# probabilists/azula

Hardware: AMD Instinct MI355X
Metric: images/sec (whole node), DDIM-64 256x256 UNet (higher is better)
Workload: dtype f32 (f16x2 split: 2 half pieces per operand, 3 partial products, f32 accumulate)

## Files before the change

azula_amd/_lib.py:

```python

from __future__ import annotations

import ctypes as C
import functools
import os
import threading

import torch

_HERE = os.path.dirname(os.path.abspath(__file__))
LIB_PATH = os.environ.get("AZULA_AMD_LIB") or os.path.join(_HERE, "csrc", "libazula_amd.so")

c_f32p = C.c_void_p
c_stream = C.c_void_p


class AzStepCoef(C.Structure):
    _fields_ = [
        ("c_in", C.c_float),
        ("c_skip", C.c_float),
        ("c_out", C.c_float),
        ("c_time", C.c_float),
        ("alpha_t", C.c_float),
        ("alpha_s", C.c_float),
# ... 412 lines not shown
    "az_rownorm_mod_f32": [vp, vp, vp, vp, vp, i64, i64, i64, i64, i64, i32, f32, c_stream],
    "az_rownorm_mod_h16": [vp, vp, vp, vp, vp, i64, i64, i64, i64, i64, i32, f32, i32, c_stream],
    "az_groupnorm_stats_h16": [vp, vp, vp, i64, i64, i64, i64, i64, i32, i32, i32, c_stream],
    "az_affine_act_h16": [vp, vp, vp, i64, vp, vp, i64, i64, i64, i64, i32, i32, i32, c_stream],
    "az_token_copy_f32": [vp, i64, i64, vp, i64, i64, i64, i64, i64, c_stream],
    "az_token_fill_f32": [vp, i64, i64, i64, vp, i64, vp, i64, i64, c_stream],
    "az_token_fill_h16": [vp, i64, i64, i64, vp, i64, vp, i64, i64, i32, c_stream],
    "az_timestep_embedding_f32": [vp, i64, vp, i64, i64, i32, f32, c_stream],
    "az_linear_small_grouped_f32": [vp, i32, i32, i64, i32, i32, c_stream],
    "az_conv2d_f32": [C.POINTER(AzConvArgs), c_stream],
    "az_conv2d_stem_f32": [C.POINTER(AzConvArgs), c_stream],
    "az_conv2d_bf16_f32": [C.POINTER(AzConvArgs), c_stream],
    "az_conv2d_x3_f32": [C.POINTER(AzConvArgs), c_stream],
    "az_conv2d_f16_f32": [C.POINTER(AzConvArgs), c_stream],
    "az_pack_conv_weight_half_f32": [vp, vp, i32, i32, i32, i32, i32, i32, i32, i32, c_stream],
    "az_pack_conv_weight_x3_f32": [vp, vp, i32, i32, i32, i32, i32, i32, i32, c_stream],
    "az_conv2d_suggest_splitk": [i64, i32, i32, i32],
    "az_conv2d_x3_suggest_splitk": [C.POINTER(AzConvArgs)],
    "az_conv2d_winograd_f32": [C.POINTER(AzConvArgs), c_stream],
    "az_conv2d_winograd_suggest_splitk": [i64, i32, i32, i32, i32],
    "az_winograd_pack_filter_f32": [vp, vp, i32, i32, i32, i32, i32, i32, c_stream],
    "az_conv2d_winograd_x3_f32": [C.POINTER(AzConvArgs), c_stream],
    "az_winograd_pack_filter_x3_f32": [vp, vp, i32, i32, i32, i32, i32, i32, c_stream],
    "az_conv2d_f16x2_f32": [C.POINTER(AzConvArgs), c_stream],
    "az_conv2d_winograd_f16x2_f32": [C.POINTER(AzConvArgs), c_stream],
    "az_pack_conv_weight_f16x2_f32": [vp, vp, i32, i32, i32, i32, i32, i32, i32, f32, c_stream],
    "az_winograd_pack_filter_f16x2_f32": [vp, vp, i32, i32, i32, i32, i32, i32, f32, c_stream],
    "az_f16x2_weight_scale": [f32, i32],
    "az_absmax_f32": [vp, vp, i64, c_stream],
    "az_absmax_from_moments_f32": [vp, vp, i64, c_stream],
    "az_conv2d_winograd4_f32": [C.POINTER(AzConvArgs), c_stream],
    "az_conv2d_winograd4_suggest_splitk": [i64, i32, i32, i32, i32],
    "az_winograd4_pack_filter_f32": [vp, vp, i32, i32, i32, i32, i32, i32, c_stream],
    "az_pack_conv_weight_f32": [vp, vp, i32, i32, i32, i32, i32, i32, i32, c_stream],
    "az_attention_f32": [C.POINTER(AzAttnArgs), c_stream],
    "az_attention_x3_f32": [C.POINTER(AzAttnArgs), c_stream],
    "az_attention_f16x2_f32": [C.POINTER(AzAttnArgs), c_stream],
    "az_attention_bf16_f32": [C.POINTER(AzAttnArgs), c_stream],
    "az_attention_f16_f32": [C.POINTER(AzAttnArgs), c_stream],
    "az_qk_prep_f32": [vp, vp, vp, vp, i64, i64, i32, i32, i64, i64, i64, i64, i64, i64, i32, i32, f32, vp, vp, c_stream],
    "az_qk_prep_bwd_f32": [vp, vp, vp, vp, vp, vp, i64, i64, i32, i32, i64, i64, i64, i64, i64, i64, i64, i64, i64, i32, i32, f32, vp, vp,
                           c_stream],
    "az_attention_bwd_f32": [C.POINTER(AzAttnBwdArgs), c_stream],
    "az_swiglu_f32": [vp, vp, i64, i64, i64, i64, c_stream],
    "az_patchify_f32": [vp, vp, vp, i64, i64, i64, i64, i64, i64, c_stream],
    "az_unpatchify_f32": [vp, vp, i64, i64, i64, i64, i64, i64, c_stream],
# ... 82 lines not shown
```

azula_amd/csrc/conv.hip:

```cpp
#include "conv_shared.h"
#include <cstdio>
#include <cstdlib>
#include <type_traits>

namespace {

constexpr int BM = 128;
constexpr int BN = 128;
constexpr int BK = 32;
constexpr int LDSS = 36;
constexpr int TILE_F = (BM + BN) * LDSS;

#include "igemm_kloop.inc"
struct ConvP {
  AzConvArgs a;
  int npix;
  int cin_s;
  int nkc0;
  int nkc1;
  int nk;
  int kps;
  int tiles_m;
  int tiles_n;
  int asm_loop;
// ... 2524 lines not shown
      else launch_igemm_half(q, half == 2, a->src_dtype != 0, dim3((unsigned)nwg, (unsigned)splitk), st);
    }
  } else
  if (half == 1 || half == 2)
    launch_igemm_half(p, half == 2, a->src_dtype != 0, dim3((unsigned)nwg, (unsigned)splitk), st);
  else if (half == 3)
    hipLaunchKernelGGL(conv_igemm_x3_kernel<false>, dim3((unsigned)nwg, (unsigned)splitk), dim3(256), 0, st, p);
  else if (half == 4)
    hipLaunchKernelGGL(conv_igemm_x3_kernel<true>, dim3((unsigned)nwg, (unsigned)splitk), dim3(256), 0, st, p);
  else if (k16)
    hipLaunchKernelGGL(conv_igemm_kernel<16>, dim3((unsigned)nwg, (unsigned)splitk), dim3(256), 0, st, p);
  else
    hipLaunchKernelGGL(conv_igemm_kernel<32>, dim3((unsigned)nwg, (unsigned)splitk), dim3(256), 0, st, p);
  int rc = az_launch_status();
  if (rc != AZ_OK) return rc;
  if (splitk > 1) {
    p.a.gn_quads = a->gn_quads;
    rc = launch_splitk_reduce(p, st, a->dst_dtype ? half : 0);
  }
  return rc;
}

static int wino_prepare(const AzConvArgs* a, int wk, int64_t ustage_bytes, WinoP& p, int& splitk);

int az_conv2d_winograd_f32(const AzConvArgs* a, az_stream_t stream) {
  WinoP p;
  int splitk = 1;
  const int prc = wino_prepare(a, WK, (int64_t)WU_STAGE * 4, p, splitk);
  if (prc != AZ_OK) return prc;
  hipStream_t st = az_s(stream);
  const int64_t nwg = (int64_t)p.cblocks * p.tblocks;
  {
    static std::atomic<uint64_t> lds_c{0}, lds_s{0};
    hipError_t e = az_max_dynamic_lds((const void*)conv_winograd_kernel<false>, W_LDS_BYTES, lds_c);
    if (e != hipSuccess) return (int)e;
    e = az_max_dynamic_lds((const void*)conv_winograd_kernel<true>, W_LDS_BYTES + W_VOFF_BYTES, lds_s);
    if (e != hipSuccess) return (int)e;
  }
  const char* asm_env = az_ab_env("AZ_WINOGRAD_ASM");
  if ((asm_env && asm_env[0] == '0') || (a->in_affine && a->in_act != 0))
    hipLaunchKernelGGL(conv_winograd_kernel<false>, dim3((unsigned)nwg, (unsigned)splitk), dim3(512), W_LDS_BYTES, st, p);
  else
    hipLaunchKernelGGL(conv_winograd_kernel<true>, dim3((unsigned)nwg, (unsigned)splitk), dim3(512), W_LDS_BYTES + W_VOFF_BYTES, st, p);
  int rc = az_launch_status();
  if (rc != AZ_OK) return rc;
  if (splitk > 1) {
    ConvP cp;
    cp.a = p.a;
    cp.a.gn_quads = a->gn_quads;
    cp.npix = p.npix;
    rc = launch_splitk_reduce(cp, st);
  }
  return rc;
}

static int winograd_x3_entry(const AzConvArgs* a, az_stream_t stream, bool h2);
int az_conv2d_winograd_x3_f32(const AzConvArgs* a, az_stream_t stream) { return winograd_x3_entry(a, stream, false); }
int az_conv2d_winograd_f16x2_f32(const AzConvArgs* a, az_stream_t stream) { return winograd_x3_entry(a, stream, true); }

static int winograd_x3_entry(const AzConvArgs* a, az_stream_t stream, bool h2) {
  WinoP p;
  int splitk = 1;
  const int prc = wino_prepare(a, 16, 16ll * WC * 16 * 3 * 2, p, splitk);
  if (prc != AZ_OK) return prc;
  AZ_REQUIRE(p.tiles_w >= 2, AZ_E_UNSUPPORTED);
  if (h2) AZ_REQUIRE(conv_pow2(a->w_scale), AZ_E_SHAPE);
  p.out_scale = h2 ? 1.f / a->w_scale : 1.f;
  if (h2) AZ_REQUIRE(AZ_ALIGNED16(a->in_absmax0) && AZ_ALIGNED16(a->in_absmax1) && (a->in_absmax0 || !a->in_absmax1), AZ_E_ALIGN);
  hipStream_t st = az_s(stream);
  int rc = azi_winograd_x3_launch(p, (unsigned)splitk, st, h2);
  if (rc != AZ_OK) return rc;
  if (splitk > 1) {
    ConvP cp;
    cp.a = p.a;
    cp.a.gn_quads = a->gn_quads;
    cp.npix = p.npix;
    rc = launch_splitk_reduce(cp, st);
  }
  return rc;
}

static int wino_prepare(const AzConvArgs* a, int wk, int64_t ustage_bytes, WinoP& p, int& splitk) {
  AZ_REQUIRE(a && a->src0 && a->weight && a->dst, AZ_E_NULL);
  AZ_REQUIRE(a->ksize == 3 && a->stride == 1 && a->pad == 1 && !a->aniso && a->src_dtype == 0 && a->dst_dtype == 0, AZ_E_UNSUPPORTED);
  AZ_REQUIRE(a->batch > 0 && a->hin > 0 && a->win > 0 && a->hout == a->hin && a->wout == a->win, AZ_E_SHAPE);
  AZ_REQUIRE(a->c0s > 0 && a->c0s % 4 == 0 && a->c1s % 4 == 0 && a->cout_s > 0 && a->cout_s % 4 == 0, AZ_E_SHAPE);
  AZ_REQUIRE((a->c1s == 0) == (a->src1 == nullptr), AZ_E_SHAPE);
  AZ_REQUIRE((a->act >= 0 && a->act <= 4) || a->act == 6, AZ_E_UNSUPPORTED);
  if (a->act == 6) AZ_REQUIRE(a->res && !a->gate && !a->dst_nchw && !a->gn_quads, AZ_E_UNSUPPORTED);
  if (a->act == 4) AZ_REQUIRE(!a->gate && !a->res && !a->dst_nchw && !a->gn_quads && a->cout_s % 8 == 0, AZ_E_UNSUPPORTED);
  if (a->depth != 0) {
    AZ_REQUIRE(a->depth > 0 && a->batch % a->depth == 0 && a->depth_shift > -a->depth && a->depth_shift < a->depth &&
                   (!a->gate || a->gate_bstride == 0) && (a->depth_wrap == 0 || a->depth_wrap == 1),
               AZ_E_UNSUPPORTED);
    const int64_t tiles_img = (int64_t)((a->hout + 1) / 2) * ((a->wout + 1) / 2);
    const int64_t span = (WT + tiles_img - 1) / tiles_img + 2 + a->depth;
    AZ_REQUIRE(span * a->h0 * a->w0 * a->c0s * 4 < (1ll << 31) && span * a->h1 * a->w1 * a->c1s * 4 < (1ll << 31), AZ_E_SHAPE);
  }
  if (a->in_affine)
    AZ_REQUIRE(!a->src1 && a->c0s % 8 == 0 && (a->up0 == 0 || wk == 16) && (a->in_act == 0 || a->in_act == 1) && AZ_ALIGNED16(a->in_affine) &&
                   (int64_t)a->batch * a->c0s * 8 < (1ll << 31),
               AZ_E_UNSUPPORTED);
// ... 25 lines not shown
  p.a = *a;
  p.npix = (int)npix64;
  p.tiles_h = (a->hout + 1) / 2;
  p.tiles_w = (a->wout + 1) / 2;
  p.ntiles = a->batch * p.tiles_h * p.tiles_w;
  p.nkc0 = (a->c0s + wk - 1) / wk;
  p.nkc1 = (a->c1s + wk - 1) / wk;
  p.nk = p.nkc0 + p.nkc1;
  {
    const int64_t tiles_img = (int64_t)p.tiles_h * p.tiles_w;
    const int64_t span = (WT + tiles_img - 1) / tiles_img + 1;
    AZ_REQUIRE(span * a->h0 * a->w0 * a->c0s * 4 < (1ll << 31), AZ_E_SHAPE);
    AZ_REQUIRE(span * a->h1 * a->w1 * a->c1s * 4 < (1ll << 31), AZ_E_SHAPE);
  }
  splitk = a->splitk;
  if (splitk > p.nk) splitk = p.nk;
  p.kps = (p.nk + splitk - 1) / splitk;
  splitk = (p.nk + p.kps - 1) / p.kps;
  p.a.splitk = splitk;
  AZ_REQUIRE(!a->gn_quads || (a->splitk == 1) == (splitk == 1), AZ_E_UNSUPPORTED);
  if (splitk > 1) p.a.gn_quads = nullptr;
  p.cblocks = (a->cout_s + WC - 1) / WC;
  p.tblocks = (p.ntiles + WT - 1) / WT;
  {
    int env_gt = 0, env_gc = 0;
    if (const char* e = az_ab_env("AZ_WINO_RECT")) sscanf(e, "%d,%d", &env_gt, &env_gc);
    int gt = env_gt > 0 ? env_gt : 8, gc = env_gt > 0 ? (env_gc > 0 ? env_gc : p.cblocks) : (wk == 16 ? 2 : 4);
    while (gc > 1 && p.cblocks % gc) gc >>= 1;
    if (env_gt <= 0) gt = 32 / gc;
    while (gt > 1 && p.tblocks % gt) gt >>= 1;
    if (p.cblocks % gc || p.tblocks % gt) gt = 1, gc = p.cblocks;
    p.gt = gt, p.gc = gc;
  }
  AZ_REQUIRE((int64_t)p.nk * p.cblocks * ustage_bytes <= (1ll << 31), AZ_E_SHAPE);
  return AZ_OK;
}

int az_conv2d_winograd_suggest_splitk(int64_t batch, int32_t hout, int32_t wout, int32_t cout_s, int32_t cin_s) {
  const int64_t tiles = batch * ((hout + 1) / 2) * ((wout + 1) / 2);
  const int64_t blocks = ((tiles + WT - 1) / WT) * ((cout_s + WC - 1) / WC);
  const int64_t nk = (cin_s + WK - 1) / WK;
  int64_t want = (256 + blocks - 1) / blocks;
  int64_t maxs = nk / 8;
  if (maxs < 1) maxs = 1;
  if (want > maxs) want = maxs;
  if (want > 16) want = 16;
  if (blocks >= 192) want = 1;
  return (int)(want < 1 ? 1 : want);
}

int az_conv2d_winograd4_f32(const AzConvArgs* a, az_stream_t stream) {
  AZ_REQUIRE(a && a->src0 && a->weight && a->dst, AZ_E_NULL);
  AZ_REQUIRE(a->ksize == 3 && a->stride == 1 && a->pad == 1 && !a->aniso && a->src_dtype == 0 && a->dst_dtype == 0, AZ_E_UNSUPPORTED);
  AZ_REQUIRE(a->batch > 0 && a->hin > 0 && a->win > 0 && a->hout == a->hin && a->wout == a->win, AZ_E_SHAPE);
  AZ_REQUIRE(a->c0s > 0 && a->c0s % 4 == 0 && a->c1s % 4 == 0 && a->cout_s > 0 && a->cout_s % 4 == 0, AZ_E_SHAPE);
  AZ_REQUIRE((a->c1s == 0) == (a->src1 == nullptr), AZ_E_SHAPE);
// ... 82 lines not shown
```

azula_amd/csrc/conv_shared.h:

```cpp
#pragma once

#include "common.h"

namespace {

typedef float f32x16 __attribute__((ext_vector_type(16)));

__device__ __forceinline__ float4 ld4(const float* p) { return *reinterpret_cast<const float4*>(p); }


typedef unsigned int u32x4 __attribute__((ext_vector_type(4)));

__device__ __forceinline__ float4 buf_ld4(__amdgpu_buffer_rsrc_t rsrc, unsigned voff, unsigned soff) {
  const u32x4 v = __builtin_amdgcn_raw_buffer_load_b128(rsrc, (int)voff, (int)soff, 0);
  return __builtin_bit_cast(float4, v);
}

typedef float f32x2 __attribute__((ext_vector_type(2)));
typedef unsigned int u32x2 __attribute__((ext_vector_type(2)));

__device__ __forceinline__ f32x2 buf_ld2(__amdgpu_buffer_rsrc_t rsrc, unsigned voff, unsigned soff) {
  const u32x2 v = __builtin_amdgcn_raw_buffer_load_b64(rsrc, (int)voff, (int)soff, 0);
  return __builtin_bit_cast(f32x2, v);
}

constexpr unsigned OOB = 0x80000000u;

__device__ __forceinline__ int wrap_coord(int i, int n, int mode) {
  if (mode) {
    i %= n;
    if (i < 0) i += n;
  }
  return i;
}
#define AZ_RSRC_CLAMP 0x80000000ll

__device__ __forceinline__ int az_depth_plane(const AzConvArgs& a, int b, bool& ok) {
  ok = true;
  if (a.depth <= 0) return b;
  const int bd = b % a.depth;
  int sb = bd + a.depth_shift;
  if (a.depth_wrap) sb = sb < 0 ? sb + a.depth : (sb >= a.depth ? sb - a.depth : sb);
  else ok = (unsigned)sb < (unsigned)a.depth;
  return b - bd + sb;
}
__device__ __forceinline__ int az_depth_base(const AzConvArgs& a, int b_first) {
  if (a.depth <= 0) return b_first;
  if (a.depth_wrap) return b_first - b_first % a.depth;
  const int s = b_first + a.depth_shift;
  return s > 0 ? s : 0;
}
// ... 253 lines not shown
    g[i] = z;
    r[i] = z;
    if (n[i] >= 0) epilogue_fetch<IO>(a, n[i], b[i], co, g[i], r[i]);
  }
#pragma unroll
  for (int i = 0; i < NB; ++i)
    if (n[i] >= 0) {
      const float4 f = epilogue_apply_store<IO>(a, n[i], b[i], co, v[i], bv, g[i], r[i]);
      if constexpr (MOM) {
        if (i == 0) mom[0] = f.x;
        const float d0 = f.x - mom[0], d1 = f.y - mom[0], d2 = f.z - mom[0], d3 = f.w - mom[0];
        mom[1] += (d0 + d1) + (d2 + d3);
        mom[2] += (d0 * d0 + d1 * d1) + (d2 * d2 + d3 * d3);
      }
    }
}

template <int IO = 0>
__device__ __forceinline__ void epilogue_store(const AzConvArgs& a, int n, int co, float4 v) {
  epilogue_store_b<IO>(a, n, n / (a.hout * a.wout), co, v);
}


}

struct WinoP {
  AzConvArgs a;
  int npix;
  int tiles_h, tiles_w, ntiles;
  int nkc0, nkc1, nk;
  int kps;
  int cblocks;
  int tblocks;
  int gt, gc;
  float out_scale;
};
```

azula_amd/csrc/wino_x3.hip:

```cpp
#include "conv_shared.h"

#include <cstdlib>
#include <type_traits>

namespace {

typedef __bf16 bf16x8 __attribute__((ext_vector_type(8)));
typedef _Float16 f16x8 __attribute__((ext_vector_type(8)));

constexpr int XT = 64;
constexpr int XC = 64;
constexpr int XK = 16;
constexpr int X_ROW = XK * 4;
constexpr int X_FREQ = XT * X_ROW;
constexpr int X_HALF = 8 * X_FREQ;
constexpr int X_STAGE = 2 * X_HALF;
constexpr int X_SLOTS = 768;
constexpr int X_SLOT = 64;
constexpr int X_DOFF1 = X_STAGE + X_SLOTS * X_SLOT;
constexpr int X_OT = 2 * XC + 4;
constexpr int X_EPI_BYTES = (4 * XT * X_OT + 3 * XT + 384) * 4;
constexpr int X_LDS_BYTES = X_DOFF1 + 512 * 32 > X_EPI_BYTES ? X_DOFF1 + 512 * 32 : X_EPI_BYTES;
static_assert(X_LDS_BYTES >= X_DOFF1 + 512 * 32 && X_LDS_BYTES >= 4 * 128 * 64 * 4, "the epilogue reuses the K loop's LDS");
constexpr int XU_STEP_BYTES = 16 * XC * XK * 3 * 2;
static_assert(4 * X_SLOTS <= 6 * 512, "six staging pieces per thread");
static_assert(X_LDS_BYTES <= 160 * 1024, "one workgroup per CU");

template <int AFF, bool TAIL, bool H2 = false>
__global__ __launch_bounds__(512, 2) void conv_winograd_x3_kernel(WinoP p) {
  extern __shared__ __attribute__((aligned(16))) float wsm[];
  char* const smem = reinterpret_cast<char*>(wsm);
  const AzConvArgs& a = p.a;
  const int tid = threadIdx.x;
  const int lane = tid & 63;
  const int wave = tid >> 6;
  const int wxi = wave & 3;
  const int wk = wave >> 2;
  const int l31 = lane & 31;
  const int h = lane >> 5;

  const int nwg = gridDim.x;
  const int bid = blockIdx.x;
  const int xq = nwg >> 3, xr = nwg & 7, xcd = bid & 7;
  const int wg = (xcd < xr ? xcd * (xq + 1) : xr * (xq + 1) + (xcd - xr) * xq) + (bid >> 3);
  const int rsz = p.gt * p.gc;
  const int rect = wg / rsz, rin = wg - rect * rsz;
  const int rcols = p.cblocks / p.gc;
  const int rrow = rect / rcols;
  const int rin_c = rin / p.gt;
  const int tb = rrow * p.gt + (rin - rin_c * p.gt);
  const int cb = (rect - rrow * rcols) * p.gc + rin_c;
  const int t0 = tb * XT;
  const int tiles_img = p.tiles_h * p.tiles_w;
  const int b_first = t0 / tiles_img;

  const int kt_begin = blockIdx.y * p.kps;
  const int kt_end = min(p.nk, kt_begin + p.kps);
  const float pin = H2 ? az_f16x2_in_scale(a.in_absmax0, a.in_absmax1, 4.f, lane) : 1.f;
  const float pin2k = pin * 2048.f;

  const int64_t s0_elems = (int64_t)a.h0 * a.w0 * a.c0s;
  const int64_t s1_elems = (int64_t)a.h1 * a.w1 * a.c1s;
  const int b_base = az_depth_base(a, b_first);
  auto clamp_bytes = [](int64_t e) { return (unsigned)(e <= 0 ? 0 : (e * 4 > AZ_RSRC_CLAMP ? AZ_RSRC_CLAMP : e * 4)); };
  const __amdgpu_buffer_rsrc_t rw = __builtin_amdgcn_make_buffer_rsrc(
      (void*)a.weight, 0, (unsigned)((int64_t)p.nk * p.cblocks * XU_STEP_BYTES), 0x00020000);
  const __amdgpu_buffer_rsrc_t rs0 = __builtin_amdgcn_make_buffer_rsrc(
      (void*)(a.src0 + b_base * s0_elems), 0, clamp_bytes((a.batch - b_base) * s0_elems), 0x00020000);
  const __amdgpu_buffer_rsrc_t rs1 = __builtin_amdgcn_make_buffer_rsrc(
      (void*)(a.src1 ? a.src1 + b_base * s1_elems : a.src0), 0, a.src1 ? clamp_bytes((a.batch - b_base) * s1_elems) : 0u, 0x00020000);

  const int vj = tid >> 3;
  const int vq = tid & 7;
  int v_b = -1, v_ih0 = 0, v_iw0 = 0;
  bool v_dok = true;
  {
    const int t = t0 + vj;
    if (t < p.ntiles) {
      const int b = t / tiles_img;
      const int r = t - b * tiles_img;
      const int th = r / p.tiles_w;
      v_b = b - b_first;
      v_ih0 = 2 * th - 1;
      v_iw0 = 2 * (r - th * p.tiles_w) - 1;
      (void)az_depth_plane(a, b, v_dok);
    }
  }
  const int tw0 = (t0 % tiles_img) % p.tiles_w;
  const int nseg = (XT - 1 + tw0) / p.tiles_w + 1;
  const int nslots = 8 * (XT + nseg);
  const int ndma = (4 * nslots + 511) >> 9;
  auto seg_of = [&](int g, int& js, int& len) {
    js = max(0, g * p.tiles_w - tw0);
    len = min(XT, (g + 1) * p.tiles_w - tw0) - js;
  };
  auto fdiv = [](int x, int d) {
    int q = (int)((float)x * __builtin_amdgcn_rcpf((float)d));
    int r = x - q * d;
    q += r >= d ? 1 : (r < 0 ? -1 : 0);
    return q;
  };
  unsigned doff[6];
  auto dma_offsets = [&](int src) {
    const int cs = src ? a.c1s : a.c0s;
    const int up = src ? a.up1 : a.up0;
    const int hs = src ? a.h1 : a.h0;
    const int ws = src ? a.w1 : a.w0;
    const int row0 = t0 / p.tiles_w;
#pragma unroll
    for (int m = 0; m < 6; ++m) {
      const int L = m * 512 + tid;
      const int s = L >> 2;
      const int g = fdiv((s >> 3) + tw0, p.tiles_w + 1);
      int js, len;
      seg_of(g, js, len);
      const int RS = 2 * len + 2;
      const int o = s - 8 * (js + g);
      const int r = fdiv(o, RS);
      const int x = o - r * RS;
      const int grow = row0 + g;
      const int b = fdiv(grow, p.tiles_h);
      const int th = grow - b * p.tiles_h;
      const int tws = g == 0 ? tw0 : 0;
      bool dok = true;
      const int bs = az_depth_plane(a, b, dok) - b_base;
      const int ih = wrap_coord(2 * th - 1 + r, a.hin, a.pad_mode);
      const int iw = wrap_coord(2 * tws - 1 + x, a.win, a.pad_mode);
      const bool ok = s < nslots && b < a.batch && dok && (unsigned)ih < (unsigned)a.hin && (unsigned)iw < (unsigned)a.win;
      doff[m] = ok ? (unsigned)((((bs * hs + (ih >> up)) * ws + (iw >> up)) * cs + (L & 3) * 4) * 4) : OOB;
    }
  };
  uint4* const park1 = reinterpret_cast<uint4*>(smem + X_DOFF1 + tid * 32);
  int cur_src = 0;
  auto switch_source = [&]() __attribute__((always_inline)) {
    cur_src = 1;
    const uint4 lo = park1[0], hi = park1[1];
    doff[0] = lo.x, doff[1] = lo.y, doff[2] = lo.z, doff[3] = lo.w, doff[4] = hi.x, doff[5] = hi.y;
  };
  if (a.src1) {
    dma_offsets(1);
    park1[0] = make_uint4(doff[0], doff[1], doff[2], doff[3]);
    park1[1] = make_uint4(doff[4], doff[5], 0u, 0u);
  }
  dma_offsets(0);
  if (kt_begin >= p.nkc0) switch_source();
  int pj_s, pj_len;
  seg_of(fdiv(vj + tw0, p.tiles_w), pj_s, pj_len);
  const int prow = (2 * pj_len + 2) * X_SLOT;
  const char* const patch = smem + X_STAGE + (8 * (pj_s + fdiv(vj + tw0, p.tiles_w)) + 2 * (vj - pj_s)) * X_SLOT + vq * 8;
  unsigned vmask = 0;
  if constexpr (AFF != 0) {
#pragma unroll
    for (int r = 0; r < 4; ++r)
#pragma unroll
      for (int c = 0; c < 4; ++c) {
        const int ih = wrap_coord(v_ih0 + r, a.hin, a.pad_mode), iw = wrap_coord(v_iw0 + c, a.win, a.pad_mode);
        if (v_b >= 0 && v_dok && (unsigned)ih < (unsigned)a.hin && (unsigned)iw < (unsigned)a.win) vmask |= 1u << (r * 4 + c);
      }
  }

  f32x2 rv[16];
  float4 gq[6];
  auto gl = [&](int kt, int m) __attribute__((always_inline)) {
    if (m < 5 || m < ndma) {
      const bool src1 = kt >= p.nkc0;
      const int kc = src1 ? kt - p.nkc0 : kt;
      const __amdgpu_buffer_rsrc_t r = src1 ? rs1 : rs0;
      unsigned off = doff[m];
      if constexpr (TAIL) off = kc * XK + (tid & 3) * 4 < (src1 ? a.c1s : a.c0s) ? off : OOB;
      gq[m] = buf_ld4(r, off, (unsigned)(kc * XK * 4));
    }
  };
  auto gs = [&](int m) __attribute__((always_inline)) {
    if (m < 5 || m < ndma) *reinterpret_cast<float4*>(smem + X_STAGE + ((m * 512 + tid) >> 2) * X_SLOT + (tid & 3) * 16) = gq[m];
  };
  auto patch_rows = [&](int kt, int r0, int r1) __attribute__((always_inline)) {
#pragma unroll
    for (int r = r0; r < r1; ++r)
#pragma unroll
      for (int c = 0; c < 4; ++c) rv[4 * r + c] = *reinterpret_cast<const f32x2*>(patch + r * prow + c * X_SLOT);
  };
  const __amdgpu_buffer_rsrc_t raf = __builtin_amdgcn_make_buffer_rsrc(
      (void*)(AFF != 0 ? a.in_affine : nullptr), 0, AFF != 0 ? (unsigned)(2 * a.batch * a.c0s * 4) : 0u, 0x00020000);
  const unsigned af_voff = (unsigned)(((b_first + (v_b < 0 ? 0 : v_b)) * a.c0s + vq * 2) * 4);
  const unsigned af_shift = (unsigned)(a.batch * a.c0s * 4);
  f32x2 af_sc = {0.f, 0.f}, af_sh = {0.f, 0.f};
  auto affine_load = [&](int kt) __attribute__((always_inline)) {
    if constexpr (AFF != 0) {
      const bool kv = !TAIL || kt * XK + vq * 2 < a.c0s;
      af_sc = buf_ld2(raf, kv ? af_voff : OOB, (unsigned)(kt * XK * 4));
      af_sh = buf_ld2(raf, kv ? af_voff : OOB, (unsigned)(kt * XK * 4) + af_shift);
    }
  };
  auto affine = [&]() __attribute__((always_inline)) {
    if constexpr (AFF != 0) {
#pragma unroll
      for (int i = 0; i < 16; ++i) {
// ... 259 lines not shown
    __syncthreads();
    if (wk == 0) {
      float* zbuf = wsm + wxi * (XT * X_OT);
#pragma unroll
      for (int th = 0; th < 2; ++th)
#pragma unroll
        for (int ch = 0; ch < 2; ++ch) {
          float* zrow = zbuf + (th * 32 + l31) * X_OT + ch * 32 + 4 * h;
          const f32x16& z0 = acc[2 * ch + th];
          const f32x16& z1 = acc[4 + 2 * ch + th];
#pragma unroll
          for (int g = 0; g < 4; ++g) {
            *reinterpret_cast<float4*>(zrow + 8 * g) = make_float4(z0[4 * g], z0[4 * g + 1], z0[4 * g + 2], z0[4 * g + 3]);
            *reinterpret_cast<float4*>(zrow + XC + 8 * g) = make_float4(z1[4 * g], z1[4 * g + 1], z1[4 * g + 2], z1[4 * g + 3]);
          }
        }
    }
  }
  int* tinfo = reinterpret_cast<int*>(wsm + 4 * XT * X_OT);
  if (wave < 2 && h == 0) {
    const int tl = wave * 32 + l31;
    const int t = t0 + tl;
    int n00 = -1, fl = 0, b = 0;
    if (t < p.ntiles) {
      b = t / tiles_img;
      const int rr = t - b * tiles_img;
      const int th = rr / p.tiles_w;
      const int tw = rr - th * p.tiles_w;
      n00 = (b * a.hout + 2 * th) * a.wout + 2 * tw;
      fl = (2 * th + 1 < a.hout ? 1 : 0) | (2 * tw + 1 < a.wout ? 2 : 0);
    }
    tinfo[tl] = n00;
    tinfo[XT + tl] = fl;
    tinfo[2 * XT + tl] = b;
  }
  __syncthreads();
  const int cq = tid & 15;
  const int co = cb * XC + cq * 4;
  if (co >= a.cout_s) return;
  int on[8], ob[8];
  float4 ov[8];
#pragma unroll
  for (int it = 0; it < 8; ++it) {
    const int row = (it * 512 + tid) >> 4;
    const int tile = row >> 2, px = row & 3;
    const int n00 = tinfo[tile], fl = tinfo[XT + tile];
    ob[it] = tinfo[2 * XT + tile];
// ... 21 lines not shown
    am = am + 0.5f * d;
    a2 = (a2 + b2) + d * d * half_n;
  };
  chan(am, a2, __shfl_xor(am, 16), __shfl_xor(a2, 16), 16.f);
  chan(am, a2, __shfl_xor(am, 32), __shfl_xor(a2, 32), 32.f);
  float* sh = reinterpret_cast<float*>(tinfo + 3 * XT);
  if (lane < 16) {
    sh[wave * 16 + lane] = am;
    sh[128 + wave * 16 + lane] = a2;
  }
  __syncthreads();
  if (tid < 16) {
    float wm[8], w2[8];
#pragma unroll
    for (int k = 0; k < 8; ++k) {
      wm[k] = sh[k * 16 + tid];
      w2[k] = sh[128 + k * 16 + tid];
    }
    float hn = 64.f;
#pragma unroll
    for (int o = 1; o < 8; o <<= 1, hn *= 2.f)
#pragma unroll
      for (int k = 0; k < 8; k += 2 * o) chan(wm[k], w2[k], wm[k + o], w2[k + o], hn);
    const int chunk = (t0 - b_first * tiles_img) / XT;
    float* out = a.gn_quads + ((((int64_t)b_first * a.gn_chunks + chunk) * (a.cout_s / 4)) + (cb * (XC / 4) + tid)) * 4;
    out[0] = 1024.f;
    out[1] = wm[0];
    out[2] = w2[0];
    out[3] = 0.f;
  }
}

}

template <int AFF, bool TAIL, bool H2>
static int launch_x3(const WinoP& p, unsigned splitk, hipStream_t st) {
  static std::atomic<uint64_t> lds_set{0};
  hipError_t e = az_max_dynamic_lds((const void*)conv_winograd_x3_kernel<AFF, TAIL, H2>, X_LDS_BYTES, lds_set);
  if (e != hipSuccess) return (int)e;
  hipLaunchKernelGGL((conv_winograd_x3_kernel<AFF, TAIL, H2>), dim3((unsigned)((int64_t)p.cblocks * p.tblocks), splitk), dim3(512), X_LDS_BYTES,
                     st, p);
  return az_launch_status();
}

template <bool H2>
static int launch_x3_mode(const WinoP& p, unsigned splitk, hipStream_t st) {
  const bool tail = (p.a.c0s % XK) != 0 || (p.a.c1s % XK) != 0;
  const int aff = !p.a.in_affine ? 0 : (p.a.in_act == 0 ? 1 : 2);
  switch (aff * 2 + (tail ? 1 : 0)) {
    case 0: return launch_x3<0, false, H2>(p, splitk, st);
    case 1: return launch_x3<0, true, H2>(p, splitk, st);
    case 2: return launch_x3<1, false, H2>(p, splitk, st);
    case 3: return launch_x3<1, true, H2>(p, splitk, st);
    case 4: return launch_x3<2, false, H2>(p, splitk, st);
    default: return launch_x3<2, true, H2>(p, splitk, st);
  }
}

__attribute__((visibility("hidden"))) int azi_winograd_x3_launch(const WinoP& p, unsigned splitk, hipStream_t st, bool h2) {
  return h2 ? launch_x3_mode<true>(p, splitk, st) : launch_x3_mode<false>(p, splitk, st);
}
```

include/azula_amd.h:

```cpp
#ifndef AZULA_AMD_H
#define AZULA_AMD_H

#include <stdint.h>

#ifdef __cplusplus
extern "C" {
#endif

#define AZ_VERSION 1

enum {
  AZ_OK = 0,
  AZ_E_NULL = -1,
  AZ_E_SHAPE = -2,
  AZ_E_ALIGN = -3,
  AZ_E_UNSUPPORTED = -4
};

typedef void* az_stream_t;

int az_version(void);
const char* az_error_string(int code);

typedef struct AzStepCoef {
// ... 314 lines not shown
  int32_t qk_rmsnorm;
  float qk_eps;
  int32_t qk_reserved;
  const float* qk_q_weight;
  const float* qk_k_weight;
  const float* qk_rope_cos;
  const float* qk_rope_sin;
  int32_t depth_wrap;
  int32_t dst_dtype;
  float w_scale;
  int32_t reserved1;
  const float* in_absmax0;
  const float* in_absmax1;
} AzConvArgs;
int az_conv2d_f32(const AzConvArgs* args, az_stream_t stream);
int az_conv2d_stem_f32(const AzConvArgs* args, az_stream_t stream);
int az_conv2d_bf16_f32(const AzConvArgs* args, az_stream_t stream);
int az_conv2d_f16_f32(const AzConvArgs* args, az_stream_t stream);
int az_conv2d_x3_f32(const AzConvArgs* args, az_stream_t stream);
int az_conv2d_x3_suggest_splitk(const AzConvArgs* args);
int az_conv2d_winograd_f32(const AzConvArgs* args, az_stream_t stream);
int az_conv2d_winograd_suggest_splitk(int64_t batch, int32_t hout, int32_t wout, int32_t cout_s, int32_t cin_s);
int az_conv2d_winograd_x3_f32(const AzConvArgs* args, az_stream_t stream);
#define AZ_F16X2_IN_SCALE 0.0625f
int az_conv2d_f16x2_f32(const AzConvArgs* args, az_stream_t stream);
int az_conv2d_winograd_f16x2_f32(const AzConvArgs* args, az_stream_t stream);
float az_f16x2_weight_scale(float amax, int32_t winograd);
#define AZ_ABSMAX_SLOTS 256
int az_absmax_f32(float* slots, const float* x, int64_t n, az_stream_t stream);
int az_absmax_from_moments_f32(float* slots, const float* partials, int64_t count, az_stream_t stream);
int az_conv2d_winograd4_f32(const AzConvArgs* args, az_stream_t stream);
int az_conv2d_winograd4_suggest_splitk(int64_t batch, int32_t hout, int32_t wout, int32_t cout_s, int32_t cin_s);
int az_conv2d_suggest_splitk(int64_t npix, int32_t cout_s, int32_t cin_s, int32_t ksize);
int az_pack_conv_weight_f32(float* dst, const float* src, int32_t cout, int32_t cin, int32_t ks, int32_t cout_s,
                            int32_t cin0, int32_t c0s, int32_t cin_s, az_stream_t stream);

typedef struct AzAttnArgs {
  const float* q;
  const float* k;
  const float* v;
  float* out;
  int32_t batch, heads, tokens, head_dim;
  int64_t q_bstride, q_tstride, q_hstride;
  int64_t k_bstride, k_tstride, k_hstride;
  int64_t v_bstride, v_tstride, v_hstride;
  int64_t o_bstride, o_tstride, o_hstride;
// ... 119 lines not shown
```

Before: 4.407.

## Add rectangular tile blocks to x3 Winograd conv to shrink halo input staging

Adds a RECT variant of the x3/f16x2 Winograd kernel where each workgroup covers a 2D rectangle of output tiles (e.g. 16x4, 8x8) instead of a 64-tile run along a row. A host-side chooser estimates the input slots each layout needs and picks the rectangle with the fewest halo pixels, which cuts global loads and LDS staging per block. It also adds geometry query entry points and an env override. The cost is more template instantiations and extra per-thread index arithmetic, and the GroupNorm chunk indexing changes under the rectangular layout.

```diff
diff --git a/azula_amd/_lib.py b/azula_amd/_lib.py
--- a/azula_amd/_lib.py
+++ b/azula_amd/_lib.py
@@ -458,6 +458,8 @@
     "az_winograd_pack_filter_f32": [vp, vp, i32, i32, i32, i32, i32, i32, c_stream],
     "az_conv2d_winograd_x3_f32": [C.POINTER(AzConvArgs), c_stream],
     "az_winograd_pack_filter_x3_f32": [vp, vp, i32, i32, i32, i32, i32, i32, c_stream],
+    "az_winograd_x3_choose_block": [i32, i32, i32, i32, vp, vp, vp, vp],
+    "az_winograd_x3_block_geometry": [i32, i32, i32, i32, i32, i32, i32, vp, vp],
     "az_conv2d_f16x2_f32": [C.POINTER(AzConvArgs), c_stream],
     "az_conv2d_winograd_f16x2_f32": [C.POINTER(AzConvArgs), c_stream],
     "az_pack_conv_weight_f16x2_f32": [vp, vp, i32, i32, i32, i32, i32, i32, i32, f32, c_stream],
diff --git a/azula_amd/csrc/conv.hip b/azula_amd/csrc/conv.hip
--- a/azula_amd/csrc/conv.hip
+++ b/azula_amd/csrc/conv.hip
@@ -2570,6 +2570,7 @@
 }
 
 static int wino_prepare(const AzConvArgs* a, int wk, int64_t ustage_bytes, WinoP& p, int& splitk);
+static void wino_order(WinoP& p, int wk);
 
 int az_conv2d_winograd_f32(const AzConvArgs* a, az_stream_t stream) {
   WinoP p;
@@ -2606,12 +2607,104 @@
 int az_conv2d_winograd_x3_f32(const AzConvArgs* a, az_stream_t stream) { return winograd_x3_entry(a, stream, false); }
 int az_conv2d_winograd_f16x2_f32(const AzConvArgs* a, az_stream_t stream) { return winograd_x3_entry(a, stream, true); }
 
+constexpr int X3_NSHAPES = 5;
+constexpr int X3_SHAPES[X3_NSHAPES][2] = {{64, 1}, {32, 2}, {16, 4}, {8, 8}, {4, 16}};
+constexpr bool X3_RECT_BLOCKS = true;
+
+static bool x3_shape_ok(int rw, int rh) {
+  for (int i = 0; i < X3_NSHAPES; ++i)
+    if (X3_SHAPES[i][0] == rw && X3_SHAPES[i][1] == rh) return true;
+  return false;
+}
+
+static int64_t x3_run_slots(int64_t ntiles, int tiles_w) {
+  const int64_t nb = (ntiles + WT - 1) / WT;
+  int g = WT, r = tiles_w;
+  while (r) { const int x = g % r; g = r; r = x; }
+  const int period = tiles_w / g;
+  int64_t total = 0;
+  for (int i = 0; i < period && i < nb; ++i) {
+    const int tw0 = (int)(((int64_t)i * WT) % tiles_w);
+    const int nseg = (WT - 1 + tw0) / tiles_w + 1;
+    total += (nb / period + (i < nb % period ? 1 : 0)) * 8 * (WT + nseg);
+  }
+  return total;
+}
+
+static int64_t x3_choose_block(int batch, int tiles_h, int tiles_w, bool whole, int& rw, int& rh, int64_t& run_slots) {
+  const int64_t ntiles = (int64_t)batch * tiles_h * tiles_w;
+  const int64_t run_blocks = (ntiles + WT - 1) / WT;
+  run_slots = x3_run_slots(ntiles, tiles_w);
+  int64_t best = run_slots;
+  rw = WT, rh = 1;
+  if (!X3_RECT_BLOCKS) return best;
+  for (int i = 1; i < X3_NSHAPES; ++i) {
+    const int w = X3_SHAPES[i][0], h = X3_SHAPES[i][1];
+    if (whole && (tiles_w % w || tiles_h % h)) continue;
+    const int64_t blocks = (int64_t)batch * x3_rect_blocks_per_image(tiles_h, tiles_w, w, h);
+    if (blocks > run_blocks) continue;
+    const int64_t slots = blocks * (2 * w + 2) * (2 * h + 2);
+    if (slots < best) best = slots, rw = w, rh = h;
+  }
+  return best;
+}
+
+int az_winograd_x3_choose_block(int32_t batch, int32_t hin, int32_t win, int32_t whole, int32_t* rect_w, int32_t* rect_h,
+                                int64_t* slots, int64_t* slots_run) {
+  AZ_REQUIRE(rect_w && rect_h && slots && slots_run, AZ_E_NULL);
+  AZ_REQUIRE(batch > 0 && hin > 0 && win > 0 && (int64_t)batch * hin * win < (1ll << 31), AZ_E_SHAPE);
+  int rw, rh;
+  int64_t run;
+  *slots = x3_choose_block(batch, (hin + 1) / 2, (win + 1) / 2, whole != 0, rw, rh, run);
+  *rect_w = rw, *rect_h = rh, *slots_run = run;
+  return AZ_OK;
+}
+
+int az_winograd_x3_block_geometry(int32_t batch, int32_t hin, int32_t win, int32_t pad_mode, int32_t rect_w, int32_t rect_h,
+                                  int32_t block, int32_t* slot_pix, int32_t* tile_info) {
+  AZ_REQUIRE(slot_pix && tile_info, AZ_E_NULL);
+  AZ_REQUIRE(batch > 0 && hin > 0 && win > 0 && (int64_t)batch * hin * win < (1ll << 31), AZ_E_SHAPE);
+  AZ_REQUIRE(rect_h > 1 && x3_shape_ok(rect_w, rect_h), AZ_E_UNSUPPORTED);
+  const int tiles_h = (hin + 1) / 2, tiles_w = (win + 1) / 2;
+  AZ_REQUIRE(block >= 0 && block < (int64_t)batch * x3_rect_blocks_per_image(tiles_h, tiles_w, rect_w, rect_h), AZ_E_SHAPE);
+  const X3RectGeom g = x3_rect_geom(block, tiles_h, tiles_w, rect_w, rect_h);
+  for (int s = 0; s < 512; ++s) {
+    int ih, iw;
+    const bool ok = x3_rect_slot_pixel(g, s, hin, win, pad_mode, ih, iw);
+    slot_pix[3 * s] = ok ? g.b : -1, slot_pix[3 * s + 1] = ok ? ih : -1, slot_pix[3 * s + 2] = ok ? iw : -1;
+  }
+  for (int j = 0; j < WT; ++j) {
+    int th, tw, ps;
+    const bool ok = x3_rect_tile(g, j, tiles_h, tiles_w, th, tw, ps);
+    tile_info[4 * j] = ok ? g.b : -1, tile_info[4 * j + 1] = th, tile_info[4 * j + 2] = tw, tile_info[4 * j + 3] = ps;
+  }
+  return g.nslots;
+}
+
 static int winograd_x3_entry(const AzConvArgs* a, az_stream_t stream, bool h2) {
   WinoP p;
   int splitk = 1;
   const int prc = wino_prepare(a, 16, 16ll * WC * 16 * 3 * 2, p, splitk);
   if (prc != AZ_OK) return prc;
   AZ_REQUIRE(p.tiles_w >= 2, AZ_E_UNSUPPORTED);
+  {
+    const bool whole = p.a.gn_quads != nullptr;
+    int rw, rh;
+    int64_t run_slots;
+    x3_choose_block(a->batch, p.tiles_h, p.tiles_w, whole, rw, rh, run_slots);
+    if (const char* e = az_ab_env("AZ_X3_BLOCK")) {
+      int ew = 0, eh = 0;
+      if (sscanf(e, "%d,%d", &ew, &eh) == 2) {
+        AZ_REQUIRE(x3_shape_ok(ew, eh) && !(whole && eh > 1 && (p.tiles_w % ew || p.tiles_h % eh)), AZ_E_UNSUPPORTED);
+        rw = ew, rh = eh;
+      }
+    }
+    if (rh > 1) {
+      p.rect_w = rw, p.rect_h = rh;
+      p.tblocks = a->batch * x3_rect_blocks_per_image(p.tiles_h, p.tiles_w, rw, rh);
+      wino_order(p, 16);
+    }
+  }
   if (h2) AZ_REQUIRE(conv_pow2(a->w_scale), AZ_E_SHAPE);
   p.out_scale = h2 ? 1.f / a->w_scale : 1.f;
   if (h2) AZ_REQUIRE(AZ_ALIGNED16(a->in_absmax0) && AZ_ALIGNED16(a->in_absmax1) && (a->in_absmax0 || !a->in_absmax1), AZ_E_ALIGN);
@@ -2626,6 +2719,17 @@
     rc = launch_splitk_reduce(cp, st);
   }
   return rc;
+}
+
+static void wino_order(WinoP& p, int wk) {
+  int env_gt = 0, env_gc = 0;
+  if (const char* e = az_ab_env("AZ_WINO_RECT")) sscanf(e, "%d,%d", &env_gt, &env_gc);
+  int gt = env_gt > 0 ? env_gt : 8, gc = env_gt > 0 ? (env_gc > 0 ? env_gc : p.cblocks) : (wk == 16 ? 2 : 4);
+  while (gc > 1 && p.cblocks % gc) gc >>= 1;
+  if (env_gt <= 0) gt = 32 / gc;
+  while (gt > 1 && p.tblocks % gt) gt >>= 1;
+  if (p.cblocks % gc || p.tblocks % gt) gt = 1, gc = p.cblocks;
+  p.gt = gt, p.gc = gc;
 }
 
 static int wino_prepare(const AzConvArgs* a, int wk, int64_t ustage_bytes, WinoP& p, int& splitk) {
@@ -2697,16 +2801,8 @@
   if (splitk > 1) p.a.gn_quads = nullptr;
   p.cblocks = (a->cout_s + WC - 1) / WC;
   p.tblocks = (p.ntiles + WT - 1) / WT;
-  {
-    int env_gt = 0, env_gc = 0;
-    if (const char* e = az_ab_env("AZ_WINO_RECT")) sscanf(e, "%d,%d", &env_gt, &env_gc);
-    int gt = env_gt > 0 ? env_gt : 8, gc = env_gt > 0 ? (env_gc > 0 ? env_gc : p.cblocks) : (wk == 16 ? 2 : 4);
-    while (gc > 1 && p.cblocks % gc) gc >>= 1;
-    if (env_gt <= 0) gt = 32 / gc;
-    while (gt > 1 && p.tblocks % gt) gt >>= 1;
-    if (p.cblocks % gc || p.tblocks % gt) gt = 1, gc = p.cblocks;
-    p.gt = gt, p.gc = gc;
-  }
+  p.rect_w = WT, p.rect_h = 1;
+  wino_order(p, wk);
   AZ_REQUIRE((int64_t)p.nk * p.cblocks * ustage_bytes <= (1ll << 31), AZ_E_SHAPE);
   return AZ_OK;
 }
diff --git a/azula_amd/csrc/conv_shared.h b/azula_amd/csrc/conv_shared.h
--- a/azula_amd/csrc/conv_shared.h
+++ b/azula_amd/csrc/conv_shared.h
@@ -26,7 +26,7 @@
 
 constexpr unsigned OOB = 0x80000000u;
 
-__device__ __forceinline__ int wrap_coord(int i, int n, int mode) {
+__host__ __device__ __forceinline__ int wrap_coord(int i, int n, int mode) {
   if (mode) {
     i %= n;
     if (i < 0) i += n;
@@ -326,6 +326,60 @@
 }
 
 
+__host__ __device__ __forceinline__ int az_fdiv(int x, int d) {
+#if defined(__HIP_DEVICE_COMPILE__)
+  int q = (int)((float)x * __builtin_amdgcn_rcpf((float)d));
+#else
+  int q = (int)((float)x / (float)d);
+#endif
+  const int r = x - q * d;
+  q += r >= d ? 1 : (r < 0 ? -1 : 0);
+  return q;
+}
+
+struct X3RectGeom {
+  int rw, rh;
+  int ws;
+  int nslots;
+  int b, rb;
+  int th0, tw0;
+};
+
+__host__ __device__ __forceinline__ int x3_rect_blocks_per_image(int tiles_h, int tiles_w, int rw, int rh) {
+  return az_fdiv(tiles_h + rh - 1, rh) * az_fdiv(tiles_w + rw - 1, rw);
+}
+
+__host__ __device__ __forceinline__ X3RectGeom x3_rect_geom(int tb, int tiles_h, int tiles_w, int rw, int rh) {
+  X3RectGeom g;
+  g.rw = rw, g.rh = rh;
+  g.ws = 2 * rw + 2;
+  g.nslots = (2 * rh + 2) * g.ws;
+  const int bw = az_fdiv(tiles_w + rw - 1, rw);
+  const int bpi = az_fdiv(tiles_h + rh - 1, rh) * bw;
+  g.b = az_fdiv(tb, bpi);
+  g.rb = tb - g.b * bpi;
+  const int by = az_fdiv(g.rb, bw);
+  g.th0 = by * rh;
+  g.tw0 = (g.rb - by * bw) * rw;
+  return g;
+}
+
+__host__ __device__ __forceinline__ bool x3_rect_slot_pixel(const X3RectGeom& g, int s, int hin, int win, int pad_mode, int& ih, int& iw) {
+  const int r = az_fdiv(s, g.ws);
+  ih = wrap_coord(2 * g.th0 - 1 + r, hin, pad_mode);
+  iw = wrap_coord(2 * g.tw0 - 1 + (s - r * g.ws), win, pad_mode);
+  return s < g.nslots && (unsigned)ih < (unsigned)hin && (unsigned)iw < (unsigned)win;
+}
+
+__host__ __device__ __forceinline__ bool x3_rect_tile(const X3RectGeom& g, int j, int tiles_h, int tiles_w, int& th, int& tw, int& pslot) {
+  const int jy = az_fdiv(j, g.rw), jx = j - jy * g.rw;
+  th = g.th0 + jy;
+  tw = g.tw0 + jx;
+  pslot = 2 * jy * g.ws + 2 * jx;
+  return th < tiles_h && tw < tiles_w;
+}
+
+
 }
 
 struct WinoP {
@@ -337,5 +391,6 @@
   int cblocks;
   int tblocks;
   int gt, gc;
+  int rect_w, rect_h;
   float out_scale;
 };
diff --git a/azula_amd/csrc/wino_x3.hip b/azula_amd/csrc/wino_x3.hip
--- a/azula_amd/csrc/wino_x3.hip
+++ b/azula_amd/csrc/wino_x3.hip
@@ -26,7 +26,7 @@
 static_assert(4 * X_SLOTS <= 6 * 512, "six staging pieces per thread");
 static_assert(X_LDS_BYTES <= 160 * 1024, "one workgroup per CU");
 
-template <int AFF, bool TAIL, bool H2 = false>
+template <int AFF, bool TAIL, bool H2 = false, bool RECT = false>
 __global__ __launch_bounds__(512, 2) void conv_winograd_x3_kernel(WinoP p) {
   extern __shared__ __attribute__((aligned(16))) float wsm[];
   char* const smem = reinterpret_cast<char*>(wsm);
@@ -52,7 +52,9 @@
   const int cb = (rect - rrow * rcols) * p.gc + rin_c;
   const int t0 = tb * XT;
   const int tiles_img = p.tiles_h * p.tiles_w;
-  const int b_first = t0 / tiles_img;
+  X3RectGeom rg = {};
+  if constexpr (RECT) rg = x3_rect_geom(tb, p.tiles_h, p.tiles_w, p.rect_w, p.rect_h);
+  const int b_first = RECT ? rg.b : t0 / tiles_img;
 
   const int kt_begin = blockIdx.y * p.kps;
   const int kt_end = min(p.nk, kt_begin + p.kps);
@@ -74,7 +76,16 @@
   const int vq = tid & 7;
   int v_b = -1, v_ih0 = 0, v_iw0 = 0;
   bool v_dok = true;
-  {
+  int v_pslot = 0;
+  if constexpr (RECT) {
+    int th, tw;
+    if (x3_rect_tile(rg, vj, p.tiles_h, p.tiles_w, th, tw, v_pslot)) {
+      v_b = 0;
+      v_ih0 = 2 * th - 1;
+      v_iw0 = 2 * tw - 1;
+      (void)az_depth_plane(a, rg.b, v_dok);
+    }
+  } else {
     const int t = t0 + vj;
     if (t < p.ntiles) {
       const int b = t / tiles_img;
@@ -88,7 +99,7 @@
   }
   const int tw0 = (t0 % tiles_img) % p.tiles_w;
   const int nseg = (XT - 1 + tw0) / p.tiles_w + 1;
-  const int nslots = 8 * (XT + nseg);
+  const int nslots = RECT ? rg.nslots : 8 * (XT + nseg);
   const int ndma = (4 * nslots + 511) >> 9;
   auto seg_of = [&](int g, int& js, int& len) {
     js = max(0, g * p.tiles_w - tw0);
@@ -111,6 +122,14 @@
     for (int m = 0; m < 6; ++m) {
       const int L = m * 512 + tid;
       const int s = L >> 2;
+      if constexpr (RECT) {
+        bool dok = true;
+        const int bs = az_depth_plane(a, rg.b, dok) - b_base;
+        int ih, iw;
+        const bool ok = x3_rect_slot_pixel(rg, s, a.hin, a.win, a.pad_mode, ih, iw) && dok;
+        doff[m] = ok ? (unsigned)((((bs * hs + (ih >> up)) * ws + (iw >> up)) * cs + (L & 3) * 4) * 4) : OOB;
+        continue;
+      }
       const int g = fdiv((s >> 3) + tw0, p.tiles_w + 1);
       int js, len;
       seg_of(g, js, len);
@@ -146,8 +165,8 @@
   if (kt_begin >= p.nkc0) switch_source();
   int pj_s, pj_len;
   seg_of(fdiv(vj + tw0, p.tiles_w), pj_s, pj_len);
-  const int prow = (2 * pj_len + 2) * X_SLOT;
-  const char* const patch = smem + X_STAGE + (8 * (pj_s + fdiv(vj + tw0, p.tiles_w)) + 2 * (vj - pj_s)) * X_SLOT + vq * 8;
+  const int prow = RECT ? rg.ws * X_SLOT : (2 * pj_len + 2) * X_SLOT;
+  const char* const patch = smem + X_STAGE + (RECT ? v_pslot : 8 * (pj_s + fdiv(vj + tw0, p.tiles_w)) + 2 * (vj - pj_s)) * X_SLOT + vq * 8;
   unsigned vmask = 0;
   if constexpr (AFF != 0) {
 #pragma unroll
@@ -162,7 +181,7 @@
   f32x2 rv[16];
   float4 gq[6];
   auto gl = [&](int kt, int m) __attribute__((always_inline)) {
-    if (m < 5 || m < ndma) {
+    if (RECT ? m < 3 || (m < 4 && m < ndma) : m < 5 || m < ndma) {
       const bool src1 = kt >= p.nkc0;
       const int kc = src1 ? kt - p.nkc0 : kt;
       const __amdgpu_buffer_rsrc_t r = src1 ? rs1 : rs0;
@@ -172,7 +191,7 @@
     }
   };
   auto gs = [&](int m) __attribute__((always_inline)) {
-    if (m < 5 || m < ndma) *reinterpret_cast<float4*>(smem + X_STAGE + ((m * 512 + tid) >> 2) * X_SLOT + (tid & 3) * 16) = gq[m];
+    if (RECT ? m < 3 || (m < 4 && m < ndma) : m < 5 || m < ndma) *reinterpret_cast<float4*>(smem + X_STAGE + ((m * 512 + tid) >> 2) * X_SLOT + (tid & 3) * 16) = gq[m];
   };
   auto patch_rows = [&](int kt, int r0, int r1) __attribute__((always_inline)) {
 #pragma unroll
@@ -478,7 +497,14 @@
     const int tl = wave * 32 + l31;
     const int t = t0 + tl;
     int n00 = -1, fl = 0, b = 0;
-    if (t < p.ntiles) {
+    if constexpr (RECT) {
+      int th, tw, ps;
+      if (x3_rect_tile(rg, tl, p.tiles_h, p.tiles_w, th, tw, ps)) {
+        b = rg.b;
+        n00 = (b * a.hout + 2 * th) * a.wout + 2 * tw;
+        fl = (2 * th + 1 < a.hout ? 1 : 0) | (2 * tw + 1 < a.wout ? 2 : 0);
+      }
+    } else if (t < p.ntiles) {
       b = t / tiles_img;
       const int rr = t - b * tiles_img;
       const int th = rr / p.tiles_w;
@@ -546,7 +572,7 @@
     for (int o = 1; o < 8; o <<= 1, hn *= 2.f)
 #pragma unroll
       for (int k = 0; k < 8; k += 2 * o) chan(wm[k], w2[k], wm[k + o], w2[k + o], hn);
-    const int chunk = (t0 - b_first * tiles_img) / XT;
+    const int chunk = RECT ? rg.rb : (t0 - b_first * tiles_img) / XT;
     float* out = a.gn_quads + ((((int64_t)b_first * a.gn_chunks + chunk) * (a.cout_s / 4)) + (cb * (XC / 4) + tid)) * 4;
     out[0] = 1024.f;
     out[1] = wm[0];
@@ -557,30 +583,34 @@
 
 }
 
-template <int AFF, bool TAIL, bool H2>
+template <int AFF, bool TAIL, bool H2, bool RECT>
 static int launch_x3(const WinoP& p, unsigned splitk, hipStream_t st) {
   static std::atomic<uint64_t> lds_set{0};
-  hipError_t e = az_max_dynamic_lds((const void*)conv_winograd_x3_kernel<AFF, TAIL, H2>, X_LDS_BYTES, lds_set);
+  hipError_t e = az_max_dynamic_lds((const void*)conv_winograd_x3_kernel<AFF, TAIL, H2, RECT>, X_LDS_BYTES, lds_set);
   if (e != hipSuccess) return (int)e;
-  hipLaunchKernelGGL((conv_winograd_x3_kernel<AFF, TAIL, H2>), dim3((unsigned)((int64_t)p.cblocks * p.tblocks), splitk), dim3(512), X_LDS_BYTES,
+  hipLaunchKernelGGL((conv_winograd_x3_kernel<AFF, TAIL, H2, RECT>), dim3((unsigned)((int64_t)p.cblocks * p.tblocks), splitk), dim3(512), X_LDS_BYTES,
                      st, p);
   return az_launch_status();
 }
 
-template <bool H2>
+template <bool H2, bool RECT>
 static int launch_x3_mode(const WinoP& p, unsigned splitk, hipStream_t st) {
   const bool tail = (p.a.c0s % XK) != 0 || (p.a.c1s % XK) != 0;
   const int aff = !p.a.in_affine ? 0 : (p.a.in_act == 0 ? 1 : 2);
   switch (aff * 2 + (tail ? 1 : 0)) {
-    case 0: return launch_x3<0, false, H2>(p, splitk, st);
-    case 1: return launch_x3<0, true, H2>(p, splitk, st);
-    case 2: return launch_x3<1, false, H2>(p, splitk, st);
-    case 3: return launch_x3<1, true, H2>(p, splitk, st);
-    case 4: return launch_x3<2, false, H2>(p, splitk, st);
-    default: return launch_x3<2, true, H2>(p, splitk, st);
+    case 0: return launch_x3<0, false, H2, RECT>(p, splitk, st);
+    case 1: return launch_x3<0, true, H2, RECT>(p, splitk, st);
+    case 2: return launch_x3<1, false, H2, RECT>(p, splitk, st);
+    case 3: return launch_x3<1, true, H2, RECT>(p, splitk, st);
+    case 4: return launch_x3<2, false, H2, RECT>(p, splitk, st);
+    default: return launch_x3<2, true, H2, RECT>(p, splitk, st);
   }
 }
 
 __attribute__((visibility("hidden"))) int azi_winograd_x3_launch(const WinoP& p, unsigned splitk, hipStream_t st, bool h2) {
-  return h2 ? launch_x3_mode<true>(p, splitk, st) : launch_x3_mode<false>(p, splitk, st);
+  if (p.rect_h > 1) {
+    if (p.rect_w * p.rect_h != XT || (2 * p.rect_w + 2) * (2 * p.rect_h + 2) > 512) return AZ_E_SHAPE;
+    return h2 ? launch_x3_mode<true, true>(p, splitk, st) : launch_x3_mode<false, true>(p, splitk, st);
+  }
+  return h2 ? launch_x3_mode<true, false>(p, splitk, st) : launch_x3_mode<false, false>(p, splitk, st);
 }
diff --git a/include/azula_amd.h b/include/azula_amd.h
--- a/include/azula_amd.h
+++ b/include/azula_amd.h
@@ -360,6 +360,10 @@
 int az_conv2d_winograd_f32(const AzConvArgs* args, az_stream_t stream);
 int az_conv2d_winograd_suggest_splitk(int64_t batch, int32_t hout, int32_t wout, int32_t cout_s, int32_t cin_s);
 int az_conv2d_winograd_x3_f32(const AzConvArgs* args, az_stream_t stream);
+int az_winograd_x3_choose_block(int32_t batch, int32_t hin, int32_t win, int32_t whole, int32_t* rect_w, int32_t* rect_h,
+                                int64_t* slots, int64_t* slots_run);
+int az_winograd_x3_block_geometry(int32_t batch, int32_t hin, int32_t win, int32_t pad_mode, int32_t rect_w, int32_t rect_h,
+                                  int32_t block, int32_t* slot_pix, int32_t* tile_info);
 #define AZ_F16X2_IN_SCALE 0.0625f
 int az_conv2d_f16x2_f32(const AzConvArgs* args, az_stream_t stream);
 int az_conv2d_winograd_f16x2_f32(const AzConvArgs* args, az_stream_t stream);
```

Result: faster. 4.742 (median of 6 runs) (+7.6%).
